# hedgepigdaniel/video-annotator

Hardware: AMD Instinct MI355X
Metric: stabilized frames/sec at 4K NV12, 1/2/4/8 GPU; remap % HBM roofline (higher is better)
Workload: dtype u8 pixels / f32 map / f64 rotations

## Files before the change

video-annotator_amd/csrc/vstab_pyramid.hip:

```cpp
#include <algorithm>

#include <hip/hip_ext.h>

#include "vstab_internal.hpp"
#include "vstab_track.hpp"
#include "vstab_track_device.hpp"

namespace vstab {

__device__ __forceinline__ uint32_t udot4(uint32_t a, uint32_t b, uint32_t c) { return __builtin_amdgcn_udot4(a, b, c, false); }

__device__ __forceinline__ uint32_t pyr_down_dot4x4(const uint32_t (&d)[5][4]) {
    uint32_t acc[4] = {128u, 128u, 128u, 128u};
#pragma unroll
    for (int j = 0; j < 5; j++) {
        const uint32_t k = j == 0 || j == 4 ? 1u : j == 2 ? 6u : 4u;
        const uint32_t w_hi2 = (k << 16) | (4 * k << 24);
        const uint32_t w_lo3 = 6 * k | (4 * k << 8) | (k << 16);
        const uint32_t w_all = k | (4 * k << 8) | (6 * k << 16) | (4 * k << 24);
        acc[0] = udot4(d[j][1], w_lo3, udot4(d[j][0], w_hi2, acc[0]));
        acc[1] = udot4(d[j][2], k, udot4(d[j][1], w_all, acc[1]));
        acc[2] = udot4(d[j][2], w_lo3, udot4(d[j][1], w_hi2, acc[2]));
        acc[3] = udot4(d[j][3], k, udot4(d[j][2], w_all, acc[3]));
    }
    const uint32_t p01 = __builtin_amdgcn_perm(acc[1], acc[0], 0x0c0c0501u), p23 = __builtin_amdgcn_perm(acc[3], acc[2], 0x0c0c0501u);
    return __builtin_amdgcn_perm(p23, p01, 0x05040100u);
}

template <bool EDGE, bool NEAR, bool COPY = false>
__device__ __forceinline__ uint32_t pyr_down_group4(const uint8_t *__restrict__ src, uint32_t spitch, int sw, int sh, int x0, int y, bool vec_ok,
                                                    uint8_t *__restrict__ cp = nullptr, uint32_t cpitch = 0) {
    const int sx0 = 2 * x0 - 4;
    const uint8_t *row[5];
#pragma unroll
    for (int j = 0; j < 5; j++) {
        const int ry = 2 * y - 2 + j;
        row[j] = src + (uint32_t)(NEAR ? min(abs(ry), 2 * sh - 2 - abs(ry)) : reflect101(ry, sh)) * spitch;
    }
    uint32_t d[5][4];
    if (!EDGE) {
        if (y >= 1 && 2 * y + 2 < sh) {
            const uint8_t *r0 = src + (size_t)(uint32_t)(2 * y - 2) * spitch + sx0;
#pragma unroll
            for (int j = 0; j < 5; j++) {
                const uint4 v = *reinterpret_cast<const uint4 *>(r0 + (size_t)j * spitch);
                d[j][0] = v.x, d[j][1] = v.y, d[j][2] = v.z, d[j][3] = v.w;
            }
        } else {
#pragma unroll
            for (int j = 0; j < 5; j++) {
                const uint32_t *p = reinterpret_cast<const uint32_t *>(row[j] + sx0);
                d[j][0] = p[0], d[j][1] = p[1], d[j][2] = p[2], d[j][3] = p[3];
            }
        }
    } else {
#pragma unroll
        for (int q = 0; q < 4; q++) {
            const int gx = sx0 + 4 * q;
            if (vec_ok && gx >= 0 && gx + 4 <= sw) {
#pragma unroll
                for (int j = 0; j < 5; j++) d[j][q] = *reinterpret_cast<const uint32_t *>(row[j] + gx);
            } else {
                int col[4];
#pragma unroll
                for (int i = 0; i < 4; i++) col[i] = NEAR ? min(abs(gx + i), 2 * sw - 2 - abs(gx + i)) : reflect101(gx + i, sw);
#pragma unroll
                for (int j = 0; j < 5; j++)
                    d[j][q] = (uint32_t)row[j][col[0]] | ((uint32_t)row[j][col[1]] << 8) | ((uint32_t)row[j][col[2]] << 16) | ((uint32_t)row[j][col[3]] << 24);
            }
        }
    }
    if (COPY) {
#pragma unroll
        for (int jj = 2; jj <= 3; jj++) {
            const int r = 2 * y + jj - 2;
            if (r >= sh) break;
            uint8_t *o = cp + (uint32_t)r * cpitch + (uint32_t)(2 * x0);
            if (!EDGE) {
                *reinterpret_cast<uint2 *>(o) = make_uint2(d[jj][1], d[jj][2]);
            } else {
#pragma unroll
                for (int b = 0; b < 8; b++)
                    if (2 * x0 + b < sw) o[b] = (uint8_t)((b < 4 ? d[jj][1] : d[jj][2]) >> (8 * (b & 3)));
            }
        }
    }
    return pyr_down_dot4x4(d);
}

template <bool EDGE, bool NEAR, bool COPY = false>
__device__ __forceinline__ void pyr_down_group(const uint8_t *__restrict__ src, uint32_t spitch, int sw, int sh, uint8_t *__restrict__ dst, size_t dpitch,
                                               int dw, int x0, int y, bool vec_ok, uint8_t *__restrict__ cp = nullptr, uint32_t cpitch = 0) {
    const uint32_t out = pyr_down_group4<EDGE, NEAR, COPY>(src, spitch, sw, sh, x0, y, vec_ok, cp, cpitch);
    uint8_t *o = dst + (size_t)((uint32_t)y * (uint32_t)dpitch) + x0;
    if (!EDGE) {
        *reinterpret_cast<uint32_t *>(o) = out;
    } else {
        for (int c = 0; c < 4 && x0 + c < dw; c++) o[c] = (uint8_t)(out >> (8 * c));
    }
}

template <bool COPY>
__device__ __forceinline__ void pyr_down_dispatch(const uint8_t *__restrict__ src, uint32_t spitch, int sw, int sh, uint8_t *__restrict__ dst, size_t dpitch, int dw,
                                                  int dh, int vec_ok, int g_lo, int g_hi, int nbx, int nb_edge, int n_groups, int near,
                                                  uint8_t *__restrict__ cp = nullptr, uint32_t cpitch = 0) {
    if ((int)blockIdx.x >= nb_edge) {
        const int b = blockIdx.x - nb_edge, by = b / nbx, bx = b - by * nbx;
        const int g = g_lo + bx * 64 + (threadIdx.x & 63), y = by * 4 + (threadIdx.x >> 6);
        if (g >= g_hi || y >= dh) return;
        pyr_down_group<false, true, COPY>(src, spitch, sw, sh, dst, dpitch, dw, 4 * g, y, true, cp, cpitch);
    } else {
        const int n_edge = n_groups - (g_hi - g_lo);
        const int e = blockIdx.x * 256 + threadIdx.x;
        const int y = e / n_edge, i = e - y * n_edge;
        if (y >= dh) return;
        const int g = i < g_lo ? i : g_hi + (i - g_lo);
        if (near)
            pyr_down_group<true, true, COPY>(src, spitch, sw, sh, dst, dpitch, dw, 4 * g, y, vec_ok != 0, cp, cpitch);
        else
            pyr_down_group<true, false, COPY>(src, spitch, sw, sh, dst, dpitch, dw, 4 * g, y, vec_ok != 0, cp, cpitch);
    }
}

__global__ void __launch_bounds__(256) k_pyr_down(const uint8_t *__restrict__ src, size_t spitch, int sw, int sh,
                                                  uint8_t *__restrict__ dst, size_t dpitch, int dw, int dh, int vec_ok, int g_lo, int g_hi,
                                                  int nbx, int nb_edge, int n_groups, int near) {
    pyr_down_dispatch<false>(src, (uint32_t)spitch, sw, sh, dst, dpitch, dw, dh, vec_ok, g_lo, g_hi, nbx, nb_edge, n_groups, near);
}

__global__ void __launch_bounds__(256) k_pack_pyr(const uint8_t *__restrict__ src, uint32_t spitch, int sw, int sh, uint8_t *__restrict__ dst, uint32_t dpitch,
                                                  int dw, int dh, int vec_ok, int g_lo, int g_hi, int nbx, int nb_edge, int n_groups, int near, int nb_pyr,
                                                  const uint8_t *__restrict__ uv, uint32_t uvpitch, uint8_t *__restrict__ ring, uint32_t rpitch, int uv_vec) {
    if ((int)blockIdx.x >= nb_pyr) {
        uint8_t *cdst = ring + (uint32_t)sh * rpitch;
        const int rows = sh / 2;
        if (uv_vec) {
            const int vecs = sw / 16;
            for (int e = ((int)blockIdx.x - nb_pyr) * 256 + threadIdx.x; e < rows * vecs; e += ((int)gridDim.x - nb_pyr) * 256) {
                const int r = e / vecs, c = e - r * vecs;
                reinterpret_cast<uint4 *>(cdst + (uint32_t)r * rpitch)[c] = reinterpret_cast<const uint4 *>(uv + (uint32_t)r * uvpitch)[c];
            }
        } else {
            for (int e = ((int)blockIdx.x - nb_pyr) * 256 + threadIdx.x; e < rows * sw; e += ((int)gridDim.x - nb_pyr) * 256) {
                const int r = e / sw, c = e - r * sw;
                cdst[(uint32_t)r * rpitch + c] = uv[(uint32_t)r * uvpitch + c];
            }
        }
        return;
    }
    pyr_down_dispatch<true>(src, spitch, sw, sh, dst, dpitch, dw, dh, vec_ok, g_lo, g_hi, nbx, nb_edge, n_groups, near, ring, rpitch);
}

constexpr int P2_TW = 16, P2_TH = 10;
constexpr int P2_MG = (2 * P2_TW + 5 + 3) / 4, P2_MW = 4 * P2_MG;
constexpr int P2_MH = 2 * P2_TH + 3;
constexpr int P2_ITEMS = P2_MG * P2_MH, P2_ROUNDS = (P2_ITEMS + 255) / 256;
static_assert(P2_TW % 4 == 0 && 2 * P2_TW + 5 <= P2_MW, "the region holds the taps of the tile's last output");

template <bool NEAR>
__device__ __forceinline__ void pyr_down_x2_tile(const uint8_t *__restrict__ src, uint32_t spitch, int sw, int sh, uint8_t *__restrict__ mid, uint32_t mpitch, int mw,
                                                 int mh, uint8_t *__restrict__ dst, uint32_t dpitch, int dw, int dh, bool vec_ok, bool dst_vec_ok,
                                                 uint8_t (&smid)[P2_MH][P2_MW]) {
    const int tid = threadIdx.x;
    const int x0 = blockIdx.x * P2_TW, y0 = blockIdx.y * P2_TH;
    const int mx0 = 2 * x0 - 4, my0 = 2 * y0 - 2;
    const bool interior = vec_ok && mx0 >= 2 && my0 >= 1 && mx0 + P2_MW <= mw && my0 + P2_MH <= mh && 2 * (mx0 + P2_MW) + 4 <= sw && 2 * (my0 + P2_MH) + 1 <= sh;
    if (interior) {
        uint32_t d[P2_ROUNDS][5][4];
#pragma unroll
        for (int k = 0; k < P2_ROUNDS; k++) {
            const int it = min(tid + 256 * k, P2_ITEMS - 1);
            const int ry = it / P2_MG, g = it - ry * P2_MG;
            const uint8_t *r0 = src + (uint32_t)(2 * (my0 + ry) - 2) * spitch + (uint32_t)(2 * (mx0 + 4 * g) - 4);
#pragma unroll
            for (int j = 0; j < 5; j++) {
                const uint4 v = *reinterpret_cast<const uint4 *>(r0 + (uint32_t)j * spitch);
                d[k][j][0] = v.x, d[k][j][1] = v.y, d[k][j][2] = v.z, d[k][j][3] = v.w;
            }
        }
#pragma unroll
        for (int k = 0; k < P2_ROUNDS; k++) {
            const int it = tid + 256 * k;
            if (it >= P2_ITEMS) break;
            const int ry = it / P2_MG, g = it - ry * P2_MG;
            const uint32_t out = pyr_down_dot4x4(d[k]);
            *reinterpret_cast<uint32_t *>(&smid[ry][4 * g]) = out;
            if (g >= 1 && g <= P2_TW / 2 && ry >= 2 && ry < 2 + 2 * P2_TH) *reinterpret_cast<uint32_t *>(mid + (uint32_t)(my0 + ry) * mpitch + (mx0 + 4 * g)) = out;
        }
    } else {
#pragma unroll 1
        for (int k = 0; k < P2_ROUNDS; k++) {
            const int it = tid + 256 * k;
            if (it >= P2_ITEMS) break;
            const int ry = it / P2_MG, g = it - ry * P2_MG;
            const int my = my0 + ry, mx = mx0 + 4 * g;
            if (my < 0 || my >= mh || mx < 0 || mx >= mw) continue;
            const uint32_t out = pyr_down_group4<true, NEAR>(src, spitch, sw, sh, mx, my, vec_ok);
            *reinterpret_cast<uint32_t *>(&smid[ry][4 * g]) = out;
            if (g >= 1 && g <= P2_TW / 2 && ry >= 2 && ry < 2 + 2 * P2_TH) {
                uint8_t *o = mid + (uint32_t)my * mpitch + mx;
                if (vec_ok && mx + 4 <= mw) *reinterpret_cast<uint32_t *>(o) = out;
                else
                    for (int c = 0; c < 4 && mx + c < mw; c++) o[c] = (uint8_t)(out >> (8 * c));
            }
        }
    }
    __syncthreads();
    if (interior) {
        if (tid < (P2_TW / 4) * P2_TH) {
            const int ty = tid / (P2_TW / 4), g = tid - ty * (P2_TW / 4);
            uint32_t d[5][4];
#pragma unroll
            for (int j = 0; j < 5; j++) {
                const uint2 lo = *reinterpret_cast<const uint2 *>(&smid[2 * ty + j][8 * g]), hi = *reinterpret_cast<const uint2 *>(&smid[2 * ty + j][8 * g + 8]);
                d[j][0] = lo.x, d[j][1] = lo.y, d[j][2] = hi.x, d[j][3] = hi.y;
            }
            const uint32_t out = pyr_down_dot4x4(d);
            uint8_t *o = dst + (uint32_t)(y0 + ty) * dpitch + (x0 + 4 * g);
            if (dst_vec_ok) *reinterpret_cast<uint32_t *>(o) = out;
            else
                for (int c = 0; c < 4; c++) o[c] = (uint8_t)(out >> (8 * c));
        }
    } else {
        for (int e = tid; e < P2_TW * P2_TH; e += 256) {
            const int ty = e / P2_TW, tx = e - ty * P2_TW;
            const int x = x0 + tx, y = y0 + ty;
            if (x >= dw || y >= dh) continue;
            int col[5];
#pragma unroll
            for (int i = 0; i < 5; i++) col[i] = reflect101(2 * x - 2 + i, mw) - mx0;
            uint32_t acc = 128u;
#pragma unroll
            for (int j = 0; j < 5; j++) {
                const uint8_t *r = smid[reflect101(2 * y - 2 + j, mh) - my0];
                const uint32_t k = j == 0 || j == 4 ? 1u : j == 2 ? 6u : 4u;
                acc += k * ((uint32_t)r[col[0]] + 4u * r[col[1]] + 6u * r[col[2]] + 4u * r[col[3]] + r[col[4]]);
            }
            dst[(uint32_t)y * dpitch + x] = (uint8_t)(acc >> 8);
        }
    }
}

__global__ void __launch_bounds__(256) k_pyr_down_x2(const uint8_t *__restrict__ src, uint32_t spitch, int sw, int sh, uint8_t *__restrict__ mid,
                                                     uint32_t mpitch, int mw, int mh, uint8_t *__restrict__ dst, uint32_t dpitch, int dw, int dh, int vec_ok,
                                                     int dst_vec_ok, int near) {
    __shared__ __attribute__((aligned(16))) uint8_t smid[P2_MH][P2_MW];
    if (near) pyr_down_x2_tile<true>(src, spitch, sw, sh, mid, mpitch, mw, mh, dst, dpitch, dw, dh, vec_ok != 0, dst_vec_ok != 0, smid);
    else pyr_down_x2_tile<false>(src, spitch, sw, sh, mid, mpitch, mw, mh, dst, dpitch, dw, dh, vec_ok != 0, dst_vec_ok != 0, smid);
}

struct PyrGrid {
    int n_groups, g_lo, g_hi, nbx, nb_int, nb_edge;
};
static PyrGrid pyr_grid(int sw, int dw, int dh, bool wide) {
    const int n_groups = div_up(dw, 4), g_lo = 1, g_hi = wide ? std::max(g_lo, std::min(sw >= 12 ? (sw - 12) / 8 + 1 : 0, dw / 4)) : g_lo;
    const int nbx = div_up(g_hi - g_lo, 64);
    return {n_groups, g_lo, g_hi, nbx, nbx * (int)div_up(dh, 4), (int)div_up(dh * (n_groups - (g_hi - g_lo)), 256)};
}

vstab_status launch_pyr_down(const uint8_t *src, size_t spitch, int sw, int sh, uint8_t *dst, size_t dpitch,
                             hipStream_t s, hipEvent_t done) {
    const int dw = (sw + 1) / 2, dh = (sh + 1) / 2;
    if ((uint64_t)spitch * (uint64_t)sh >= (1ull << 32) || (uint64_t)dpitch * (uint64_t)dh >= (1ull << 32))
        return fail(VSTAB_ERR_INVALID, "pyr_down: planes of 4 GiB or more are not supported");
    const int vec_ok = reinterpret_cast<uintptr_t>(src) % 4 == 0 && spitch % 4 == 0 && reinterpret_cast<uintptr_t>(dst) % 4 == 0 && dpitch % 4 == 0;
    const int near = sw >= 16 && sh >= 4;
    const PyrGrid g = pyr_grid(sw, dw, dh, vec_ok && near);
    hipExtLaunchKernelGGL(k_pyr_down, dim3(g.nb_edge + g.nb_int), dim3(256), 0, s, nullptr, done, 0, src, spitch, sw, sh, dst, dpitch, dw, dh, vec_ok, g.g_lo, g.g_hi, g.nbx,
                          g.nb_edge, g.n_groups, near);
    VSTAB_HIP_TRY(hipGetLastError());
    return VSTAB_OK;
}

bool pack_pyr_ok(const void *y, size_t pitch_y, const void *uv, size_t pitch_uv, int w, int h, const void *ring, const void *dst, size_t dpitch) {
    return w >= 16 && h >= 4 && !(w & 7) && !(h & 1) && reinterpret_cast<uintptr_t>(y) % 4 == 0 && pitch_y % 4 == 0 && reinterpret_cast<uintptr_t>(ring) % 8 == 0 &&
           reinterpret_cast<uintptr_t>(dst) % 4 == 0 && dpitch % 4 == 0 && pitch_y < (1u << 24) && pitch_uv < (1u << 24) && (uint64_t)pitch_y * (uint64_t)h < (1ull << 32) &&
           (uint64_t)pitch_uv * (uint64_t)(h / 2) < (1ull << 32) &&
           (uint64_t)w * (uint64_t)h * 3 / 2 < (1ull << 32);
}
vstab_status launch_pack_pyr(const uint8_t *y, size_t pitch_y, const uint8_t *uv, size_t pitch_uv, int sw, int sh, uint8_t *ring, uint8_t *dst, size_t dpitch,
                             hipStream_t s, hipEvent_t copied) {
    const int dw = (sw + 1) / 2, dh = (sh + 1) / 2;
    if (!pack_pyr_ok(y, pitch_y, uv, pitch_uv, sw, sh, ring, dst, dpitch)) return fail(VSTAB_ERR_INVALID, "pack_pyr: planes not aligned for the fused copy");
    const PyrGrid g = pyr_grid(sw, dw, dh, true);
    const int uv_vec = reinterpret_cast<uintptr_t>(uv) % 16 == 0 && pitch_uv % 16 == 0 && sw % 16 == 0 && reinterpret_cast<uintptr_t>(ring) % 16 == 0;
    const int nb_uv = std::max(1, std::min(256, (int)div_up((unsigned)(sw * (sh / 2)), 256u * 16u)));
    hipExtLaunchKernelGGL(k_pack_pyr, dim3(g.nb_edge + g.nb_int + nb_uv), dim3(256), 0, s, nullptr, copied, 0, y, (uint32_t)pitch_y, sw, sh, dst, (uint32_t)dpitch, dw, dh, 1,
                          g.g_lo, g.g_hi, g.nbx, g.nb_edge, g.n_groups, 1, g.nb_edge + g.nb_int, uv, (uint32_t)pitch_uv, ring, (uint32_t)sw, uv_vec);
    VSTAB_HIP_TRY(hipGetLastError());
    return VSTAB_OK;
}

bool pyr_down_x2_ok(int sw, int sh) { return (sw + 1) / 2 >= 8 && (sh + 1) / 2 >= 8; }
vstab_status launch_pyr_down_x2(const uint8_t *src, size_t spitch, int sw, int sh, uint8_t *mid, size_t mpitch, uint8_t *dst, size_t dpitch, hipStream_t s,
                                hipEvent_t done) {
    const int mw = (sw + 1) / 2, mh = (sh + 1) / 2, dw = (mw + 1) / 2, dh = (mh + 1) / 2;
    if (!pyr_down_x2_ok(sw, sh)) return fail(VSTAB_ERR_INVALID, "pyr_down_x2: image too small");
    if ((uint64_t)spitch * (uint64_t)sh >= (1ull << 32) || (uint64_t)mpitch * (uint64_t)mh >= (1ull << 32) || (uint64_t)dpitch * (uint64_t)dh >= (1ull << 32))
        return fail(VSTAB_ERR_INVALID, "pyr_down_x2: planes of 4 GiB or more are not supported");
    const int vec_ok = reinterpret_cast<uintptr_t>(src) % 4 == 0 && spitch % 4 == 0 && reinterpret_cast<uintptr_t>(mid) % 4 == 0 && mpitch % 4 == 0;
    const int dst_vec_ok = reinterpret_cast<uintptr_t>(dst) % 4 == 0 && dpitch % 4 == 0;
    const int near = sw >= 16 && sh >= 4;
    hipExtLaunchKernelGGL(k_pyr_down_x2, dim3(div_up(dw, P2_TW), div_up(dh, P2_TH)), dim3(256), 0, s, nullptr, done, 0, src, (uint32_t)spitch, sw, sh, mid,
                          (uint32_t)mpitch, mw, mh, dst, (uint32_t)dpitch, dw, dh, vec_ok, dst_vec_ok, near);
    VSTAB_HIP_TRY(hipGetLastError());
    return VSTAB_OK;
}

vstab_status preload_pyramid_kernels() {
    hipFuncAttributes at;
    VSTAB_HIP_TRY(hipFuncGetAttributes(&at, reinterpret_cast<const void *>(&k_pyr_down)));
    return VSTAB_OK;
}

}
```

Measured before the change: 31820.

## Compute multiple pyramid output rows per interior thread with shared row loads

Interior threads of the pyramid downsample kernels now produce R output rows each, loading 2R+3 source rows once and reusing them across the overlapping 5-tap vertical windows. The horizontal sums are computed once per source row with packed 16-bit lanes, and the vertical filter is applied with plain adds. This cuts redundant source-row loads and dot-product work. The EDGE template path is merged into the generic edge code, and the grid now scales by rows per thread. The trade is more registers per thread and fewer threads in flight.

Measured after the change: 32270 (median of 3 runs). No clear change (+1.4%).

```diff
diff --git a/video-annotator_amd/csrc/vstab_pyramid.hip b/video-annotator_amd/csrc/vstab_pyramid.hip
--- a/video-annotator_amd/csrc/vstab_pyramid.hip
+++ b/video-annotator_amd/csrc/vstab_pyramid.hip
@@ -27,7 +27,7 @@
     return __builtin_amdgcn_perm(p23, p01, 0x05040100u);
 }
 
-template <bool EDGE, bool NEAR, bool COPY = false>
+template <bool NEAR, bool COPY = false>
 __device__ __forceinline__ uint32_t pyr_down_group4(const uint8_t *__restrict__ src, uint32_t spitch, int sw, int sh, int x0, int y, bool vec_ok,
                                                     uint8_t *__restrict__ cp = nullptr, uint32_t cpitch = 0) {
     const int sx0 = 2 * x0 - 4;
@@ -38,36 +38,19 @@
         row[j] = src + (uint32_t)(NEAR ? min(abs(ry), 2 * sh - 2 - abs(ry)) : reflect101(ry, sh)) * spitch;
     }
     uint32_t d[5][4];
-    if (!EDGE) {
-        if (y >= 1 && 2 * y + 2 < sh) {
-            const uint8_t *r0 = src + (size_t)(uint32_t)(2 * y - 2) * spitch + sx0;
-#pragma unroll
-            for (int j = 0; j < 5; j++) {
-                const uint4 v = *reinterpret_cast<const uint4 *>(r0 + (size_t)j * spitch);
-                d[j][0] = v.x, d[j][1] = v.y, d[j][2] = v.z, d[j][3] = v.w;
-            }
+#pragma unroll
+    for (int q = 0; q < 4; q++) {
+        const int gx = sx0 + 4 * q;
+        if (vec_ok && gx >= 0 && gx + 4 <= sw) {
+#pragma unroll
+            for (int j = 0; j < 5; j++) d[j][q] = *reinterpret_cast<const uint32_t *>(row[j] + gx);
         } else {
-#pragma unroll
-            for (int j = 0; j < 5; j++) {
-                const uint32_t *p = reinterpret_cast<const uint32_t *>(row[j] + sx0);
-                d[j][0] = p[0], d[j][1] = p[1], d[j][2] = p[2], d[j][3] = p[3];
-            }
-        }
-    } else {
-#pragma unroll
-        for (int q = 0; q < 4; q++) {
-            const int gx = sx0 + 4 * q;
-            if (vec_ok && gx >= 0 && gx + 4 <= sw) {
-#pragma unroll
-                for (int j = 0; j < 5; j++) d[j][q] = *reinterpret_cast<const uint32_t *>(row[j] + gx);
-            } else {
-                int col[4];
-#pragma unroll
-                for (int i = 0; i < 4; i++) col[i] = NEAR ? min(abs(gx + i), 2 * sw - 2 - abs(gx + i)) : reflect101(gx + i, sw);
-#pragma unroll
-                for (int j = 0; j < 5; j++)
-                    d[j][q] = (uint32_t)row[j][col[0]] | ((uint32_t)row[j][col[1]] << 8) | ((uint32_t)row[j][col[2]] << 16) | ((uint32_t)row[j][col[3]] << 24);
-            }
+            int col[4];
+#pragma unroll
+            for (int i = 0; i < 4; i++) col[i] = NEAR ? min(abs(gx + i), 2 * sw - 2 - abs(gx + i)) : reflect101(gx + i, sw);
+#pragma unroll
+            for (int j = 0; j < 5; j++)
+                d[j][q] = (uint32_t)row[j][col[0]] | ((uint32_t)row[j][col[1]] << 8) | ((uint32_t)row[j][col[2]] << 16) | ((uint32_t)row[j][col[3]] << 24);
         }
     }
     if (COPY) {
@@ -76,27 +59,83 @@
             const int r = 2 * y + jj - 2;
             if (r >= sh) break;
             uint8_t *o = cp + (uint32_t)r * cpitch + (uint32_t)(2 * x0);
-            if (!EDGE) {
-                *reinterpret_cast<uint2 *>(o) = make_uint2(d[jj][1], d[jj][2]);
-            } else {
-#pragma unroll
-                for (int b = 0; b < 8; b++)
-                    if (2 * x0 + b < sw) o[b] = (uint8_t)((b < 4 ? d[jj][1] : d[jj][2]) >> (8 * (b & 3)));
-            }
+#pragma unroll
+            for (int b = 0; b < 8; b++)
+                if (2 * x0 + b < sw) o[b] = (uint8_t)((b < 4 ? d[jj][1] : d[jj][2]) >> (8 * (b & 3)));
         }
     }
     return pyr_down_dot4x4(d);
 }
 
-template <bool EDGE, bool NEAR, bool COPY = false>
+template <bool NEAR, bool COPY = false>
 __device__ __forceinline__ void pyr_down_group(const uint8_t *__restrict__ src, uint32_t spitch, int sw, int sh, uint8_t *__restrict__ dst, size_t dpitch,
                                                int dw, int x0, int y, bool vec_ok, uint8_t *__restrict__ cp = nullptr, uint32_t cpitch = 0) {
-    const uint32_t out = pyr_down_group4<EDGE, NEAR, COPY>(src, spitch, sw, sh, x0, y, vec_ok, cp, cpitch);
+    const uint32_t out = pyr_down_group4<NEAR, COPY>(src, spitch, sw, sh, x0, y, vec_ok, cp, cpitch);
     uint8_t *o = dst + (size_t)((uint32_t)y * (uint32_t)dpitch) + x0;
-    if (!EDGE) {
-        *reinterpret_cast<uint32_t *>(o) = out;
+    for (int c = 0; c < 4 && x0 + c < dw; c++) o[c] = (uint8_t)(out >> (8 * c));
+}
+
+#ifndef VSTAB_PYR_ROWS
+#define VSTAB_PYR_ROWS 4
+#endif
+constexpr int PYR_R = VSTAB_PYR_ROWS;
+static_assert(PYR_R == 2 || PYR_R == 4 || PYR_R == 8, "rows per interior thread");
+#ifndef VSTAB_PACK_ROWS
+#define VSTAB_PACK_ROWS 1
+#endif
+constexpr int PACK_R = VSTAB_PACK_ROWS;
+
+__device__ __forceinline__ void pyr_row_sums(const uint4 v, uint32_t &p01, uint32_t &p23) {
+    const uint32_t w_hi2 = 0x04010000u, w_lo3 = 0x00010406u, w_all = 0x04060401u;
+    const uint32_t h0 = udot4(v.y, w_lo3, udot4(v.x, w_hi2, 8u));
+    const uint32_t h1 = udot4(v.z, 1u, udot4(v.y, w_all, 8u));
+    const uint32_t h2 = udot4(v.z, w_lo3, udot4(v.y, w_hi2, 8u));
+    const uint32_t h3 = udot4(v.w, 1u, udot4(v.z, w_all, 8u));
+    p01 = h0 | (h1 << 16), p23 = h2 | (h3 << 16);
+}
+
+__device__ __forceinline__ uint32_t pyr_col_sum(uint32_t p0, uint32_t p1, uint32_t p2, uint32_t p3, uint32_t p4) {
+    return (p0 + p4) + ((p1 + p3 + p2) << 2) + (p2 << 1);
+}
+
+template <int R, bool COPY, bool FULL>
+__device__ __forceinline__ void pyr_down_rows(const uint8_t *__restrict__ src, uint32_t spitch, int sh, uint8_t *__restrict__ dst, uint32_t dpitch, int dh, int g,
+                                              int yb, uint8_t *__restrict__ cp, uint32_t cpitch) {
+    constexpr int NR = 2 * R + 3;
+    const int ry0 = 2 * yb - 2;
+    uint32_t roff[NR];
+    if (ry0 >= 0 && ry0 + NR <= sh) {
+        roff[0] = (uint32_t)ry0 * spitch;
+#pragma unroll
+        for (int j = 1; j < NR; j++) roff[j] = roff[j - 1] + spitch;
     } else {
-        for (int c = 0; c < 4 && x0 + c < dw; c++) o[c] = (uint8_t)(out >> (8 * c));
+#pragma unroll
+        for (int j = 0; j < NR; j++) roff[j] = (uint32_t)max(min(abs(ry0 + j), 2 * sh - 2 - abs(ry0 + j)), 0) * spitch;
+    }
+    const uint32_t sx0 = 8u * (uint32_t)g - 4u;
+    uint4 v[NR];
+#pragma unroll
+    for (int j = 0; j < NR; j++) v[j] = *reinterpret_cast<const uint4 *>(src + (roff[j] + sx0));
+    __builtin_amdgcn_sched_barrier(0);
+    if (!FULL) {
+#pragma unroll
+        for (int j = 0; j < NR; j++) asm volatile("" : "+v"(v[j].x), "+v"(v[j].y), "+v"(v[j].z), "+v"(v[j].w));
+    }
+    const int nrows = FULL ? R : dh - yb;
+    uint32_t p01[NR], p23[NR];
+#pragma unroll
+    for (int j = 0; j < NR; j++) pyr_row_sums(v[j], p01[j], p23[j]);
+    if (COPY) {
+        __builtin_amdgcn_sched_barrier(0);
+#pragma unroll
+        for (int j = 2; j < 2 + 2 * R; j++)
+            if ((j - 2) / 2 < nrows) *reinterpret_cast<uint2 *>(cp + ((uint32_t)(ry0 + j) * cpitch + 8u * (uint32_t)g)) = make_uint2(v[j].y, v[j].z);
+    }
+#pragma unroll
+    for (int i = 0; i < R; i++) {
+        const uint32_t r01 = pyr_col_sum(p01[2 * i], p01[2 * i + 1], p01[2 * i + 2], p01[2 * i + 3], p01[2 * i + 4]);
+        const uint32_t r23 = pyr_col_sum(p23[2 * i], p23[2 * i + 1], p23[2 * i + 2], p23[2 * i + 3], p23[2 * i + 4]);
+        if (i < nrows) *reinterpret_cast<uint32_t *>(dst + ((uint32_t)(yb + i) * dpitch + 4u * (uint32_t)g)) = __builtin_amdgcn_perm(r23, r01, 0x07050301u);
     }
 }
 
@@ -105,10 +144,13 @@
                                                   int dh, int vec_ok, int g_lo, int g_hi, int nbx, int nb_edge, int n_groups, int near,
                                                   uint8_t *__restrict__ cp = nullptr, uint32_t cpitch = 0) {
     if ((int)blockIdx.x >= nb_edge) {
+        constexpr int R = COPY ? PACK_R : PYR_R;
         const int b = blockIdx.x - nb_edge, by = b / nbx, bx = b - by * nbx;
-        const int g = g_lo + bx * 64 + (threadIdx.x & 63), y = by * 4 + (threadIdx.x >> 6);
-        if (g >= g_hi || y >= dh) return;
-        pyr_down_group<false, true, COPY>(src, spitch, sw, sh, dst, dpitch, dw, 4 * g, y, true, cp, cpitch);
+        const int wave = __builtin_amdgcn_readfirstlane(threadIdx.x >> 6);
+        const int g = g_lo + bx * 64 + (threadIdx.x & 63), yb = (by * 4 + wave) * R;
+        if (g >= g_hi || yb >= dh) return;
+        if (yb + R <= dh) pyr_down_rows<R, COPY, true>(src, spitch, sh, dst, (uint32_t)dpitch, dh, g, yb, cp, cpitch);
+        else pyr_down_rows<R, COPY, false>(src, spitch, sh, dst, (uint32_t)dpitch, dh, g, yb, cp, cpitch);
     } else {
         const int n_edge = n_groups - (g_hi - g_lo);
         const int e = blockIdx.x * 256 + threadIdx.x;
@@ -116,9 +158,9 @@
         if (y >= dh) return;
         const int g = i < g_lo ? i : g_hi + (i - g_lo);
         if (near)
-            pyr_down_group<true, true, COPY>(src, spitch, sw, sh, dst, dpitch, dw, 4 * g, y, vec_ok != 0, cp, cpitch);
+            pyr_down_group<true, COPY>(src, spitch, sw, sh, dst, dpitch, dw, 4 * g, y, vec_ok != 0, cp, cpitch);
         else
-            pyr_down_group<true, false, COPY>(src, spitch, sw, sh, dst, dpitch, dw, 4 * g, y, vec_ok != 0, cp, cpitch);
+            pyr_down_group<false, COPY>(src, spitch, sw, sh, dst, dpitch, dw, 4 * g, y, vec_ok != 0, cp, cpitch);
     }
 }
 
@@ -195,7 +237,7 @@
             const int ry = it / P2_MG, g = it - ry * P2_MG;
             const int my = my0 + ry, mx = mx0 + 4 * g;
             if (my < 0 || my >= mh || mx < 0 || mx >= mw) continue;
-            const uint32_t out = pyr_down_group4<true, NEAR>(src, spitch, sw, sh, mx, my, vec_ok);
+            const uint32_t out = pyr_down_group4<NEAR>(src, spitch, sw, sh, mx, my, vec_ok);
             *reinterpret_cast<uint32_t *>(&smid[ry][4 * g]) = out;
             if (g >= 1 && g <= P2_TW / 2 && ry >= 2 && ry < 2 + 2 * P2_TH) {
                 uint8_t *o = mid + (uint32_t)my * mpitch + mx;
@@ -252,10 +294,10 @@
 struct PyrGrid {
     int n_groups, g_lo, g_hi, nbx, nb_int, nb_edge;
 };
-static PyrGrid pyr_grid(int sw, int dw, int dh, bool wide) {
+static PyrGrid pyr_grid(int sw, int dw, int dh, bool wide, int rows) {
     const int n_groups = div_up(dw, 4), g_lo = 1, g_hi = wide ? std::max(g_lo, std::min(sw >= 12 ? (sw - 12) / 8 + 1 : 0, dw / 4)) : g_lo;
     const int nbx = div_up(g_hi - g_lo, 64);
-    return {n_groups, g_lo, g_hi, nbx, nbx * (int)div_up(dh, 4), (int)div_up(dh * (n_groups - (g_hi - g_lo)), 256)};
+    return {n_groups, g_lo, g_hi, nbx, nbx * (int)div_up(dh, 4 * rows), (int)div_up(dh * (n_groups - (g_hi - g_lo)), 256)};
 }
 
 vstab_status launch_pyr_down(const uint8_t *src, size_t spitch, int sw, int sh, uint8_t *dst, size_t dpitch,
@@ -265,7 +307,7 @@
         return fail(VSTAB_ERR_INVALID, "pyr_down: planes of 4 GiB or more are not supported");
     const int vec_ok = reinterpret_cast<uintptr_t>(src) % 4 == 0 && spitch % 4 == 0 && reinterpret_cast<uintptr_t>(dst) % 4 == 0 && dpitch % 4 == 0;
     const int near = sw >= 16 && sh >= 4;
-    const PyrGrid g = pyr_grid(sw, dw, dh, vec_ok && near);
+    const PyrGrid g = pyr_grid(sw, dw, dh, vec_ok && near, PYR_R);
     hipExtLaunchKernelGGL(k_pyr_down, dim3(g.nb_edge + g.nb_int), dim3(256), 0, s, nullptr, done, 0, src, spitch, sw, sh, dst, dpitch, dw, dh, vec_ok, g.g_lo, g.g_hi, g.nbx,
                           g.nb_edge, g.n_groups, near);
     VSTAB_HIP_TRY(hipGetLastError());
@@ -282,7 +324,7 @@
                              hipStream_t s, hipEvent_t copied) {
     const int dw = (sw + 1) / 2, dh = (sh + 1) / 2;
     if (!pack_pyr_ok(y, pitch_y, uv, pitch_uv, sw, sh, ring, dst, dpitch)) return fail(VSTAB_ERR_INVALID, "pack_pyr: planes not aligned for the fused copy");
-    const PyrGrid g = pyr_grid(sw, dw, dh, true);
+    const PyrGrid g = pyr_grid(sw, dw, dh, true, PACK_R);
     const int uv_vec = reinterpret_cast<uintptr_t>(uv) % 16 == 0 && pitch_uv % 16 == 0 && sw % 16 == 0 && reinterpret_cast<uintptr_t>(ring) % 16 == 0;
     const int nb_uv = std::max(1, std::min(256, (int)div_up((unsigned)(sw * (sh / 2)), 256u * 16u)));
     hipExtLaunchKernelGGL(k_pack_pyr, dim3(g.nb_edge + g.nb_int + nb_uv), dim3(256), 0, s, nullptr, copied, 0, y, (uint32_t)pitch_y, sw, sh, dst, (uint32_t)dpitch, dw, dh, 1,
```
